# ayankele/dune-transformercvn

Hardware: AMD Instinct MI355X
Metric: events/sec (fwd+bwd) at batch=32, 8 prongs/event; fraction of MFMA roofline (higher is better)
Workload: dtype bf16; 1 GPU; TransformerCVN DenseNet [3,6,12,6,3] g32, fwd+loss+bwd, batch 32/GPU, 8 prongs/event, 3x400x280 maps, 6-layer encoder, dropout 0.1; global_batch=32, parallelism=dp1, precision=bf16

## Files before the change

### dune-transformercvn_amd/csrc/bwd1x1_fused.hip

```cpp
#include "tcvn_ops.h"
#include "prof.h"

namespace tcvn {

namespace {

constexpr int ROWS = 64;
constexpr int TILE = ROWS * 256;
constexpr int CLD = 132;
constexpr int OFF_E = 0;
constexpr int OFF_X = TILE;
constexpr int OFF_Y = 2 * TILE;
constexpr int OFF_C = 2 * TILE;
constexpr int OFF_TAB = OFF_C + ROWS * CLD * 4;
constexpr int SMEM_BYTES = OFF_TAB + 5 * 128 * 4;

typedef __attribute__((ext_vector_type(4))) short s16x4;

__device__ __forceinline__ bf16x8_t tr_frag(const char* smem_base, int off_lo, int off_hi) {
    typedef __attribute__((address_space(3))) s16x4* lds_p;
    const s16x4 lo = __builtin_amdgcn_ds_read_tr16_b64_v4i16((lds_p)(smem_base + off_lo));
    const s16x4 hi = __builtin_amdgcn_ds_read_tr16_b64_v4i16((lds_p)(smem_base + off_hi));
    struct { s16x4 a, b; } pr = {lo, hi};
    return __builtin_bit_cast(bf16x8_t, pr);
}

__device__ __forceinline__ void dma64(char* smem_base, int buf_off, const bf16* __restrict__ A, long lda, int K, int k0, long m0, long M,
                                      const char* __restrict__ zeros, int wave, int lane) {
    const int rsub = lane >> 4, slot = lane & 15;
#pragma unroll
    for (int i = 0; i < ROWS / 16; ++i) {
        const int rg = wave + 4 * i;
        const int r = rg * 4 + rsub;
        const int col = k0 + ((slot ^ swz16(r)) << 3);
        const long m = m0 + r;
        const char* src = (m < M && col < K) ? reinterpret_cast<const char*>(A + m * lda + col) : zeros + (slot << 4);
        __builtin_amdgcn_global_load_lds((const __attribute__((address_space(1))) void*)src,
                                         (__attribute__((address_space(3))) void*)(smem_base + buf_off + rg * 1024), 16, 0, 0);
    }
}

__global__ __launch_bounds__(256, 2) void k_bwd1x1_fused_bf16(const Bwd1x1Args g) {
    extern __shared__ __attribute__((aligned(16))) char smem[];
    float* Cs = reinterpret_cast<float*>(smem + OFF_C);
    double* red = reinterpret_cast<double*>(smem + OFF_C);
    float* csum = reinterpret_cast<float*>(smem + OFF_C + 4 * 128 * 3 * 8);
    float* tab = reinterpret_cast<float*>(smem + OFF_TAB);

    const int tid = threadIdx.x;
    const int N = g.cin, n0 = blockIdx.y * 128;
    const bf16* __restrict__ DU = reinterpret_cast<const bf16*>(g.DU);
    const bf16* __restrict__ Yp = reinterpret_cast<const bf16*>(g.Y);
    const bf16* __restrict__ Xp = reinterpret_cast<const bf16*>(g.Xin);
    bf16* __restrict__ Gp = reinterpret_cast<bf16*>(g.Gout);
    const char* __restrict__ zeros = reinterpret_cast<const char*>(g.zeros);
    const long mtiles = (g.M + ROWS - 1) / ROWS;
    const u16x8 z8 = {0, 0, 0, 0, 0, 0, 0, 0};

    const bool wave_live = n0 + (tid >> 6) * 32 < N;
    bf16x8_t bw[8];
    {
        const bf16* __restrict__ Wf = reinterpret_cast<const bf16*>(g.Wfrag) + (((long)(blockIdx.y * 4 + (tid >> 6)) * 8) * 64 + (tid & 63)) * 8;
#pragma unroll
        for (int i = 0; i < 8; ++i) {
            if (wave_live) bw[i] = *reinterpret_cast<const bf16x8_t*>(Wf + (long)i * 512);
            else
#pragma unroll
                for (int j = 0; j < 8; ++j) bw[i][j] = (__bf16)0.f;
        }
    }
    if (tid < 128) {
        const bool ok = n0 + tid < N;
        tab[tid] = g.PY[tid]; tab[128 + tid] = g.QY[tid];
        tab[256 + tid] = ok ? g.sc[n0 + tid] : 0.f; tab[384 + tid] = ok ? g.sh[n0 + tid] : 0.f; tab[512 + tid] = ok ? g.sl[n0 + tid] : 0.f;
    }
    float st1[8], st2[8], st3[8], cs[8];
#pragma unroll
    for (int j = 0; j < 8; ++j) { st1[j] = 0.f; st2[j] = 0.f; st3[j] = 0.f; cs[j] = 0.f; }
    const bool wj_live = n0 + ((tid >> 6) & 1) * 64 < N;
    f32x16 accW[2][2];
#pragma unroll
    for (int a = 0; a < 2; ++a)
#pragma unroll
        for (int b = 0; b < 2; ++b)
#pragma unroll
            for (int e = 0; e < 16; ++e) accW[a][b][e] = 0.f;

    const int col_chunk = tid & 15;
    const bool col_ok = n0 + col_chunk * 8 < N;
    const int col_rem = N - (n0 + col_chunk * 8);
    const int d_r0 = (tid >> 6) * 4 + ((tid & 63) >> 4);
    const int d_chunk = (tid & 15) ^ swz16(d_r0);
    const bool xchunk_ok = n0 + (d_chunk << 3) < N;
    const unsigned voffA = (unsigned)(d_r0 * 256 + (d_chunk << 4));
    const unsigned voffX = (unsigned)(d_r0 * (int)g.ldx * 2 + (d_chunk << 4));
    const unsigned voffG = (unsigned)(((tid >> 4) * (int)g.ldg + n0 + col_chunk * 8) * 2);
    if (!xchunk_ok) {
#pragma unroll
        for (int i = 0; i < ROWS / 16; ++i) *reinterpret_cast<u16x8*>(smem + OFF_X + ((tid >> 6) + 4 * i) * 1024 + (tid & 63) * 16) = z8;
    }
    u16x8 pgv[ROWS / 16];
#pragma unroll
    for (int i = 0; i < ROWS / 16; ++i) pgv[i] = z8;
    auto request = [&](long t) {
        const long m0 = t * ROWS;
        const int wave = tid >> 6, lane = tid & 63;
        if (m0 + ROWS <= g.M) {
            const char* bE = reinterpret_cast<const char*>(DU) + m0 * 256;
            const char* bY = reinterpret_cast<const char*>(Yp) + m0 * 256;
            const char* bX = reinterpret_cast<const char*>(Xp) + (m0 * g.ldx + n0) * 2;
            const char* bG = reinterpret_cast<const char*>(Gp) + m0 * g.ldg * 2;
#pragma unroll
            for (int i = 0; i < ROWS / 16; ++i)
                __builtin_amdgcn_global_load_lds((const __attribute__((address_space(1))) void*)(bE + i * 4096 + voffA),
                                                 (__attribute__((address_space(3))) void*)(smem + OFF_E + (wave + 4 * i) * 1024), 16, 0, 0);
#pragma unroll
            for (int i = 0; i < ROWS / 16; ++i)
                __builtin_amdgcn_global_load_lds((const __attribute__((address_space(1))) void*)(bY + i * 4096 + voffA),
                                                 (__attribute__((address_space(3))) void*)(smem + OFF_Y + (wave + 4 * i) * 1024), 16, 0, 0);
            if (xchunk_ok) {
#pragma unroll
                for (int i = 0; i < ROWS / 16; ++i)
                    __builtin_amdgcn_global_load_lds((const __attribute__((address_space(1))) void*)(bX + (long)i * 32 * g.ldx + voffX),
                                                     (__attribute__((address_space(3))) void*)(smem + OFF_X + (wave + 4 * i) * 1024), 16, 0, 0);
            }
            if (col_ok) {
#pragma unroll
                for (int i = 0; i < ROWS / 16; ++i) pgv[i] = *reinterpret_cast<const u16x8*>(bG + (long)i * 32 * g.ldg + voffG);
            }
        } else {
            dma64(smem, OFF_E, DU, 128, 128, 0, m0, g.M, zeros, wave, lane);
            dma64(smem, OFF_Y, Yp, 128, 128, 0, m0, g.M, zeros, wave, lane);
            if (xchunk_ok) dma64(smem, OFF_X, Xp, g.ldx, N, n0, m0, g.M, zeros, wave, lane);
            if (col_ok) {
#pragma unroll
                for (int i = 0; i < ROWS / 16; ++i) {
                    const long m = m0 + (tid >> 4) + 16 * i;
                    if (m < g.M) pgv[i] = *reinterpret_cast<const u16x8*>(Gp + m * g.ldg + n0 + col_chunk * 8);
                }
            }
        }
    };

    long mt = blockIdx.x;
    if (mt < mtiles) request(mt);
    for (; mt < mtiles; mt += gridDim.x) {
        const long m0 = mt * ROWS;
        asm volatile("s_waitcnt vmcnt(0)" ::: "memory");
        __syncthreads();
        int t_o = tid;
        asm volatile("" : "+v"(t_o));
        const int c8 = t_o & 15, c_r0 = t_o >> 4;
        const int e_off = c_r0 * 256 + ((c8 ^ swz16(c_r0)) << 4);
        auto tab8 = [&](int which, float (&v)[8]) {
            const float4 a = *reinterpret_cast<const float4*>(tab + which * 128 + c8 * 8), b = *reinterpret_cast<const float4*>(tab + which * 128 + c8 * 8 + 4);
            v[0] = a.x; v[1] = a.y; v[2] = a.z; v[3] = a.w; v[4] = b.x; v[5] = b.y; v[6] = b.z; v[7] = b.w;
        };
        {
            float pP[8], pQ[8];
            tab8(0, pP); tab8(1, pQ);
#pragma unroll
            for (int i = 0; i < ROWS / 16; ++i) {
                const int off = e_off + i * 4096;
                const u16x8 dv = *reinterpret_cast<const u16x8*>(smem + OFF_E + off);
                const u16x8 yv = *reinterpret_cast<const u16x8*>(smem + OFF_Y + off);
                const bool live = m0 + c_r0 + 16 * i < g.M;
                u16x8 o;
#pragma unroll
                for (int j = 0; j < 8; ++j) {
                    const float t = eff3(bf2f(dv[j]), pP[j], bf2f(yv[j]), pQ[j]);
                    o[j] = live ? f2bf(t) : (bf16)0;
                    cs[j] += bf2f(o[j]);
                }
                *reinterpret_cast<u16x8*>(smem + OFF_E + off) = o;
            }
        }
        __syncthreads();
        {
            const int lane = t_o & 63, wave = t_o >> 6;
            const int r = lane & 31, h = lane >> 5;
            f32x16 acc[2];
#pragma unroll
            for (int i = 0; i < 2; ++i)
#pragma unroll
                for (int e = 0; e < 16; ++e) acc[i][e] = 0.f;
            if (wave_live) {
                const int a_base = OFF_E + r * 256, w4 = (h ^ swz16(r)) << 4;
                auto afrag = [&](int ks, int i) {
                    return *reinterpret_cast<const bf16x8_t*>(smem + a_base + i * 8192 + (w4 ^ (ks << 5)));
                };
                bf16x8_t a0 = afrag(0, 0), a1 = afrag(0, 1);
#pragma unroll
                for (int ks = 0; ks < 8; ++ks) {
                    bf16x8_t b0 = a0, b1 = a1;
                    if (ks + 1 < 8) { b0 = afrag(ks + 1, 0); b1 = afrag(ks + 1, 1); }
                    acc[0] = __builtin_amdgcn_mfma_f32_32x32x16_bf16(a0, bw[ks], acc[0], 0, 0, 0);
                    acc[1] = __builtin_amdgcn_mfma_f32_32x32x16_bf16(a1, bw[ks], acc[1], 0, 0, 0);
                    a0 = b0; a1 = b1;
                    __builtin_amdgcn_sched_barrier(0);
                }
            }
            float* cw = Cs + 4 * h * CLD + wave * 32 + r;
#pragma unroll
            for (int i = 0; i < 2; ++i)
#pragma unroll
                for (int e = 0; e < 16; ++e) cw[(i * 32 + (e & 3) + 8 * (e >> 2)) * CLD] = acc[i][e];
        }
        __syncthreads();
        if (col_ok) {
            float csc[8], csh[8], csl[8];
            tab8(2, csc); tab8(3, csh); tab8(4, csl);
            const float* crow = Cs + c_r0 * CLD + c8 * 8;
            char* gbase = reinterpret_cast<char*>(Gp) + m0 * g.ldg * 2;
#pragma unroll
            for (int i = 0; i < ROWS / 16; ++i) {
                if (m0 + c_r0 + 16 * i < g.M) {
                    const int xoff = OFF_X + e_off + i * 4096;
                    u16x8 xv = *reinterpret_cast<const u16x8*>(smem + xoff);
                    if (col_rem < 8) {
#pragma unroll
                        for (int j = 0; j < 8; ++j) xv[j] = j < col_rem ? xv[j] : (bf16)0;
                    }
                    const float4 ca = *reinterpret_cast<const float4*>(crow + i * 16 * CLD);
                    const float4 cc = *reinterpret_cast<const float4*>(crow + i * 16 * CLD + 4);
                    const float cv[8] = {ca.x, ca.y, ca.z, ca.w, cc.x, cc.y, cc.z, cc.w};
                    const u16x8 gv = pgv[i];
                    u16x8 o, xa;
#pragma unroll
                    for (int j = 0; j < 8; ++j) {
                        const float x = bf2f(xv[j]);
                        const float u = fmaf(x, csc[j], csh[j]);
                        const float dA = cv[j];
                        const float du = u > 0.f ? dA : csl[j] * dA;
                        st1[j] += du; st2[j] = fmaf(du, x, st2[j]); st3[j] = fmaf(u > 0.f ? 0.f : dA, u, st3[j]);
                        o[j] = f2bf(fmaf(csc[j], du, bf2f(gv[j])));
                        xa[j] = f2bf(prelu(u, csl[j]));
                    }
                    if (col_rem >= 8) *reinterpret_cast<u16x8*>(gbase + (long)i * 32 * g.ldg + voffG) = o;
                    else {
                        bf16* gp = reinterpret_cast<bf16*>(gbase + (long)i * 32 * g.ldg + voffG);
#pragma unroll
                        for (int j = 0; j < 8; ++j)
                            if (j < col_rem) gp[j] = o[j];
                    }
                    *reinterpret_cast<u16x8*>(smem + xoff) = xa;
                }
            }
        }
        __syncthreads();
        if (wj_live) {
            const int lane = t_o & 63, wave = t_o >> 6;
            const int wi = wave >> 1, wj = wave & 1;
            const int gq = lane >> 4, tq = (lane >> 2) & 3, tp = lane & 3;
            const int khalf = gq >> 1, chalf = gq & 1;
            const int sub = (tp & 1) * 8;
            const int rl = 8 * khalf + tq;
            int a_lo[2], a_hi[2], b_lo[2], b_hi[2];
#pragma unroll
            for (int t = 0; t < 2; ++t) {
                const int ac = wi * 8 + t * 4 + 2 * chalf + (tp >> 1), bc = wj * 8 + t * 4 + 2 * chalf + (tp >> 1);
                a_lo[t] = OFF_E + rl * 256 + ((ac ^ swz16(rl)) << 4) + sub; a_hi[t] = OFF_E + (rl + 4) * 256 + ((ac ^ swz16(rl + 4)) << 4) + sub;
                b_lo[t] = OFF_X + rl * 256 + ((bc ^ swz16(rl)) << 4) + sub; b_hi[t] = OFF_X + (rl + 4) * 256 + ((bc ^ swz16(rl + 4)) << 4) + sub;
            }
#pragma unroll
            for (int ks = 0; ks < ROWS / 16; ++ks) {
                bf16x8_t a[2], b[2];
#pragma unroll
                for (int t = 0; t < 2; ++t) {
                    a[t] = tr_frag(smem, a_lo[t] + ks * 4096, a_hi[t] + ks * 4096);
                    b[t] = tr_frag(smem, b_lo[t] + ks * 4096, b_hi[t] + ks * 4096);
                }
#pragma unroll
                for (int ta = 0; ta < 2; ++ta)
#pragma unroll
                    for (int tb = 0; tb < 2; ++tb) accW[ta][tb] = __builtin_amdgcn_mfma_f32_32x32x16_bf16(a[ta], b[tb], accW[ta][tb], 0, 0, 0);
                __builtin_amdgcn_sched_barrier(0);
            }
        }
        __syncthreads();
        if (mt + gridDim.x < mtiles) request(mt + gridDim.x);
    }
    asm volatile("s_waitcnt vmcnt(0)" ::: "memory");

    const int lane = tid & 63, wave = tid >> 6, c8 = tid & 15;
#pragma unroll
    for (int j = 0; j < 8; ++j) {
        double d1 = (double)st1[j], d2 = (double)st2[j], d3 = (double)st3[j];
        float c1 = cs[j];
        d1 += __shfl_xor(d1, 16); d1 += __shfl_xor(d1, 32);
        d2 += __shfl_xor(d2, 16); d2 += __shfl_xor(d2, 32);
        d3 += __shfl_xor(d3, 16); d3 += __shfl_xor(d3, 32);
        c1 += __shfl_xor(c1, 16); c1 += __shfl_xor(c1, 32);
        if (lane < 16) {
            double* p = red + ((wave * 128) + c8 * 8 + j) * 3;
            p[0] = d1; p[1] = d2; p[2] = d3;
            csum[wave * 128 + c8 * 8 + j] = c1;
        }
    }
    __syncthreads();
    if (tid < 128) {
        if (n0 + tid < N) {
            double a = 0, b = 0, c = 0;
#pragma unroll
            for (int w = 0; w < 4; ++w) { a += red[(w * 128 + tid) * 3]; b += red[(w * 128 + tid) * 3 + 1]; c += red[(w * 128 + tid) * 3 + 2]; }
            double* p = g.part + ((long)blockIdx.x * N + n0 + tid) * 3;
            p[0] = a; p[1] = b; p[2] = c;
        }
        if (blockIdx.y == 0) g.tail[(long)blockIdx.x * 128 + tid] = (csum[tid] + csum[128 + tid]) + (csum[256 + tid] + csum[384 + tid]);
    }
    const int wi = wave >> 1, wj = wave & 1;
    const int cj = lane & 31, hh = lane >> 5;
#pragma unroll
    for (int ta = 0; ta < 2; ++ta)
#pragma unroll
        for (int tb = 0; tb < 2; ++tb) {
            const int j = n0 + wj * 64 + tb * 32 + cj;
            if (j >= g.ldc) continue;
#pragma unroll
            for (int e = 0; e < 16; ++e) {
                const int i = wi * 64 + ta * 32 + (e & 3) + 8 * (e >> 2) + 4 * hh;
                g.slab[((long)blockIdx.x * 128 + i) * g.ldc + j] = accW[ta][tb][e];
            }
        }
}

}

bool bwd1x1_fused_ok(const Bwd1x1Args& a) {
    if (!a.DU || !a.Y || !a.Xin || !a.Gout || !a.Wfrag || !a.zeros || !a.part || !a.slab || !a.tail) return false;
    if (a.cin <= 0 || a.Kp != 128 || (a.ldx & 7) || (a.ldg & 7) || a.ldc < a.cin || a.ldc > cdiv(a.cin, 128) * 128) return false;
    const uintptr_t al = reinterpret_cast<uintptr_t>(a.DU) | reinterpret_cast<uintptr_t>(a.Y) | reinterpret_cast<uintptr_t>(a.Xin) |
                         reinterpret_cast<uintptr_t>(a.Gout) | reinterpret_cast<uintptr_t>(a.Wfrag) | reinterpret_cast<uintptr_t>(a.slab);
    if (al & 15) return false;
    return (long)bwd1x1_fused_nblk(a) * 128 * a.ldc * 4 <= a.slab_bytes;
}

int bwd1x1_fused_nblk(const Bwd1x1Args& a) {
    const int nn = cdiv(a.cin, 128);
    int cap = 512 / nn;
    if (cap < 64) cap = 64;
    const long mt = (a.M + ROWS - 1) / ROWS;
    return (int)(mt < cap ? mt : cap);
}

int bwd1x1_fused_launch(const Bwd1x1Args& a, hipStream_t st) {
    if (a.M <= 0) return 0;
    if (!bwd1x1_fused_ok(a)) return -2;
    if (a.nblk != bwd1x1_fused_nblk(a)) { fprintf(stderr, "tcvn: bwd1x1_fused nblk mismatch\n"); return -3; }
    static bool attr = false;
    if (!attr) {
        TCVN_CHECK(hipFuncSetAttribute(reinterpret_cast<const void*>(k_bwd1x1_fused_bf16), hipFuncAttributeMaxDynamicSharedMemorySize, 160 * 1024));
        attr = true;
    }
    ProfScope ps("k_bwd1x1_fused_bf16", 4.0 * a.M * 128.0 * a.cin, (double)a.M * (512.0 + 4.0 * a.cin), st);
    hipLaunchKernelGGL(k_bwd1x1_fused_bf16, dim3(a.nblk, cdiv(a.cin, 128)), dim3(256), SMEM_BYTES, st, a);
    TCVN_LAUNCH_CHECK();
    return 0;
}

int bwd1x1_fused_reduce(const Bwd1x1Args& a, float* dWk, float* dbias, const SlabJob* extra, hipStream_t st, const BnBwdLinkArgs* link) {
    SlabJob jobs[4] = {};
    if (a.M > 0) { jobs[0] = slab_job(a.slab, a.nblk, 128L * a.ldc, dWk, 0); jobs[1] = slab_job(a.tail, a.nblk, 128, dbias, 0); }
    if (extra != nullptr) { jobs[2] = extra[0]; jobs[3] = extra[1]; }
    if (link != nullptr) return slab_reduce4_link(jobs, 4, *link, st);
    return slab_reduce4(jobs, 4, st);
}

}
```

### dune-transformercvn_amd/csrc/fwd1x1_fused.hip

```cpp
#include "tcvn_ops.h"
#include "prof.h"

namespace tcvn {

namespace {

constexpr int ROWS = 64;
constexpr int TILE = ROWS * 256;
constexpr int CLD = 136;

template <int NKC> struct FwdCfg {
    static constexpr int OFF_C = NKC * TILE;
    static constexpr int OFF_TAB = OFF_C + ROWS * CLD * 2;
    static constexpr int SMEM = OFF_TAB + 3 * NKC * 128 * 4;
};

template <int NKC, bool OACT>
__global__ __launch_bounds__(256, 3) void k_fwd1x1_fused_bf16(const Fwd1x1Args g) {
    extern __shared__ __attribute__((aligned(16))) char smem[];
    typedef FwdCfg<NKC> C;
    constexpr int KS = NKC * 8;
    bf16* Cs = reinterpret_cast<bf16*>(smem + C::OFF_C);
    double* red = reinterpret_cast<double*>(smem);
    float* tab = reinterpret_cast<float*>(smem + C::OFF_TAB);

    const int tid = threadIdx.x;
    const int K = g.cin;
    const bf16* __restrict__ Xp = reinterpret_cast<const bf16*>(g.Xin);
    const char* __restrict__ zeros = reinterpret_cast<const char*>(g.zeros);
    const long mtiles = (g.M + ROWS - 1) / ROWS;
    const int ksteps = g.Kp >> 4;
    const u16x8 z8 = {0, 0, 0, 0, 0, 0, 0, 0};

    bf16x8_t bw[KS];
    {
        const bf16* __restrict__ Wf = reinterpret_cast<const bf16*>(g.Wfrag) + (((long)(tid >> 6) * ksteps) * 64 + (tid & 63)) * 8;
#pragma unroll
        for (int i = 0; i < KS; ++i) {
            if (i < ksteps) bw[i] = *reinterpret_cast<const bf16x8_t*>(Wf + (long)i * 512);
            else
#pragma unroll
                for (int j = 0; j < 8; ++j) bw[i][j] = (__bf16)0.f;
        }
    }
    for (int i = tid; i < NKC * 128; i += 256) {
        const bool ok = i < K;
        float tsc = 0.f, tsh = 0.f;
        if (ok) {
            if (g.lf.isum != nullptr) lf_table(g.lf, i, blockIdx.x == 0, tsc, tsh);
            else { tsc = g.sc[i]; tsh = g.sh[i]; }
        }
        tab[i] = tsc; tab[NKC * 128 + i] = tsh; tab[2 * NKC * 128 + i] = ok ? g.sl[i] : 0.f;
    }
    const int ocol = (tid >> 6) * 32 + (tid & 31);
    const float cbias = g.bias[ocol];
    const float o_sc = OACT ? g.osc[ocol] : 1.f, o_sh = OACT ? g.osh[ocol] : 0.f, o_sl = OACT ? g.osl[ocol] : 1.f;
    float st1[8], st2[8];
#pragma unroll
    for (int j = 0; j < 8; ++j) { st1[j] = 0.f; st2[j] = 0.f; }

    const int d_r0 = (tid >> 6) * 4 + ((tid & 63) >> 4);
    const int d_chunk = (tid & 15) ^ (d_r0 & 15);
    const unsigned voffX = (unsigned)(d_r0 * (int)g.ldx * 2 + (d_chunk << 4));
#pragma unroll
    for (int kc = 0; kc < NKC; ++kc)
        if (kc * 128 + (d_chunk << 3) >= K) {
#pragma unroll
            for (int i = 0; i < ROWS / 16; ++i) *reinterpret_cast<u16x8*>(smem + kc * TILE + ((tid >> 6) + 4 * i) * 1024 + (tid & 63) * 16) = z8;
        }
    auto request = [&](long t) {
        const long m0 = t * ROWS;
        const int wave = tid >> 6, lane = tid & 63;
        if (m0 + ROWS <= g.M) {
            const char* bX = reinterpret_cast<const char*>(Xp) + m0 * g.ldx * 2;
#pragma unroll
            for (int kc = 0; kc < NKC; ++kc)
                if (kc * 128 + (d_chunk << 3) < K) {
#pragma unroll
                    for (int i = 0; i < ROWS / 16; ++i)
                        __builtin_amdgcn_global_load_lds((const __attribute__((address_space(1))) void*)(bX + kc * 256 + (long)i * 32 * g.ldx + voffX),
                                                         (__attribute__((address_space(3))) void*)(smem + kc * TILE + (wave + 4 * i) * 1024), 16, 0, 0);
                }
        } else {
            const int rsub = lane >> 4, slot = lane & 15;
#pragma unroll
            for (int kc = 0; kc < NKC; ++kc)
                if (kc * 128 + (d_chunk << 3) < K) {
#pragma unroll
                    for (int i = 0; i < ROWS / 16; ++i) {
                        const int rg = wave + 4 * i;
                        const long m = m0 + rg * 4 + rsub;
                        const char* src = m < g.M ? reinterpret_cast<const char*>(Xp + m * g.ldx + kc * 128 + (d_chunk << 3)) : zeros + (slot << 4);
                        __builtin_amdgcn_global_load_lds((const __attribute__((address_space(1))) void*)src,
                                                         (__attribute__((address_space(3))) void*)(smem + kc * TILE + rg * 1024), 16, 0, 0);
                    }
                }
        }
    };

    long mt = blockIdx.x;
    if (mt < mtiles) request(mt);
    for (; mt < mtiles; mt += gridDim.x) {
        const long m0 = mt * ROWS;
        asm volatile("s_waitcnt vmcnt(0)" ::: "memory");
        __syncthreads();
        int t_o = tid;
        asm volatile("" : "+v"(t_o));
        const int c8 = t_o & 15, c_r0 = t_o >> 4;
        const int e_off = c_r0 * 256 + ((c8 ^ (c_r0 & 15)) << 4);
#pragma unroll
        for (int kc = 0; kc < NKC; ++kc) {
            const int col = kc * 128 + c8 * 8;
            if (col < K) {
                const float* tp = tab + col;
                const float4 s0 = *reinterpret_cast<const float4*>(tp), s1 = *reinterpret_cast<const float4*>(tp + 4);
                const float4 h0 = *reinterpret_cast<const float4*>(tp + NKC * 128), h1 = *reinterpret_cast<const float4*>(tp + NKC * 128 + 4);
                const float4 l0 = *reinterpret_cast<const float4*>(tp + 2 * NKC * 128), l1 = *reinterpret_cast<const float4*>(tp + 2 * NKC * 128 + 4);
                const float sc[8] = {s0.x, s0.y, s0.z, s0.w, s1.x, s1.y, s1.z, s1.w};
                const float sh[8] = {h0.x, h0.y, h0.z, h0.w, h1.x, h1.y, h1.z, h1.w};
                const float sl[8] = {l0.x, l0.y, l0.z, l0.w, l1.x, l1.y, l1.z, l1.w};
                const int nrem = K - col;
#pragma unroll
                for (int i = 0; i < ROWS / 16; ++i) {
                    u16x8* p = reinterpret_cast<u16x8*>(smem + kc * TILE + e_off + i * 4096);
                    const u16x8 v = *p;
                    u16x8 o;
#pragma unroll
                    for (int j = 0; j < 8; ++j) o[j] = j < nrem ? f2bf(prelu(fmaf(bf2f(v[j]), sc[j], sh[j]), sl[j])) : (bf16)0;
                    *p = o;
                }
            }
        }
        __syncthreads();
        const int lane = t_o & 63, wave = t_o >> 6;
        const int r = lane & 31, h = lane >> 5;
        f32x16 acc[2];
#pragma unroll
        for (int i = 0; i < 2; ++i)
#pragma unroll
            for (int e = 0; e < 16; ++e) acc[i][e] = 0.f;
        {
            const int a_base = r * 256, w4 = (h ^ (r & 15)) << 4;
            auto afrag = [&](int s, int i) {
                return *reinterpret_cast<const bf16x8_t*>(smem + (s >> 3) * TILE + a_base + i * 8192 + (w4 ^ ((s & 7) << 5)));
            };
            bf16x8_t a0 = afrag(0, 0), a1 = afrag(0, 1);
#pragma unroll
            for (int s = 0; s < KS; ++s) {
                if (s < ksteps) {
                    bf16x8_t b0 = a0, b1 = a1;
                    if (s + 1 < KS && s + 1 < ksteps) { b0 = afrag(s + 1, 0); b1 = afrag(s + 1, 1); }
                    acc[0] = __builtin_amdgcn_mfma_f32_32x32x16_bf16(a0, bw[s], acc[0], 0, 0, 0);
                    acc[1] = __builtin_amdgcn_mfma_f32_32x32x16_bf16(a1, bw[s], acc[1], 0, 0, 0);
                    a0 = b0; a1 = b1;
                }
                __builtin_amdgcn_sched_barrier(0);
            }
        }
        __syncthreads();
        if (mt + gridDim.x < mtiles) request(mt + gridDim.x);
        {
            bf16* cw = Cs + 4 * h * CLD + wave * 32 + r;
#pragma unroll
            for (int i = 0; i < 2; ++i)
#pragma unroll
                for (int e = 0; e < 16; ++e) {
                    float v = acc[i][e] + cbias;
                    if (OACT) v = prelu(fmaf(v, o_sc, o_sh), o_sl);
                    cw[(i * 32 + (e & 3) + 8 * (e >> 2)) * CLD] = f2bf(v);
                }
        }
        __syncthreads();
        {
            const bf16* crow = Cs + c_r0 * CLD + c8 * 8;
            bf16* yb = reinterpret_cast<bf16*>(g.Out) + (m0 + c_r0) * 128 + c8 * 8;
#pragma unroll
            for (int i = 0; i < ROWS / 16; ++i) {
                if (m0 + c_r0 + 16 * i < g.M) {
                    const u16x8 o = *reinterpret_cast<const u16x8*>(crow + i * 16 * CLD);
#pragma unroll
                    for (int j = 0; j < 8; ++j) {
                        const float x = bf2f(o[j]);
                        st1[j] += x; st2[j] += x * x;
                    }
                    *reinterpret_cast<u16x8*>(yb + (long)i * 16 * 128) = o;
                }
            }
        }
    }
    asm volatile("s_waitcnt vmcnt(0)" ::: "memory");
    if (g.part == nullptr && g.isum_out == nullptr) return;
    __syncthreads();
    const int lane = tid & 63, wave = tid >> 6, c8 = tid & 15;
#pragma unroll
    for (int j = 0; j < 8; ++j) {
        double d1 = (double)st1[j], d2 = (double)st2[j];
        d1 += __shfl_xor(d1, 16); d1 += __shfl_xor(d1, 32);
        d2 += __shfl_xor(d2, 16); d2 += __shfl_xor(d2, 32);
        if (lane < 16) {
            double* p = red + ((wave * 128) + c8 * 8 + j) * 2;
            p[0] = d1; p[1] = d2;
        }
    }
    __syncthreads();
    if (tid < 128) {
        double a = 0, b = 0;
#pragma unroll
        for (int w = 0; w < 4; ++w) { a += red[(w * 128 + tid) * 2]; b += red[(w * 128 + tid) * 2 + 1]; }
        if (g.isum_out != nullptr) lf_add(g.isum_out, g.isum_stride, tid, a, b);
        else { double* p = g.part + ((long)blockIdx.x * 128 + tid) * 2; p[0] = a; p[1] = b; }
    }
}

struct WideCfg {
    static constexpr int NSLOT = 3;
    static constexpr int OFF_C = NSLOT * TILE;
    static constexpr int OFF_TAB = OFF_C + ROWS * CLD * 2;
    static constexpr int SMEM = OFF_TAB + 3 * 512 * 4;
};

template <bool OACT>
__global__ __launch_bounds__(256, 2) void k_fwd1x1_wide_bf16(const Fwd1x1Args g) {
    extern __shared__ __attribute__((aligned(16))) char smem[];
    constexpr int KS = 32;
    bf16* Cs = reinterpret_cast<bf16*>(smem + WideCfg::OFF_C);
    double* red = reinterpret_cast<double*>(smem);
    float* tab = reinterpret_cast<float*>(smem + WideCfg::OFF_TAB);

    const int tid = threadIdx.x;
    const int K = g.cin, nkc = (K + 127) >> 7;
    const bf16* __restrict__ Xp = reinterpret_cast<const bf16*>(g.Xin);
    const char* __restrict__ zeros = reinterpret_cast<const char*>(g.zeros);
    const long mtiles = (g.M + ROWS - 1) / ROWS;
    const int ksteps = g.Kp >> 4;

    for (int i = tid; i < 512; i += 256) {
        const bool ok = i < K;
        float tsc = 0.f, tsh = 0.f;
        if (ok) {
            if (g.lf.isum != nullptr) lf_table(g.lf, i, blockIdx.x == 0, tsc, tsh);
            else { tsc = g.sc[i]; tsh = g.sh[i]; }
        }
        tab[i] = tsc; tab[512 + i] = tsh; tab[1024 + i] = ok ? g.sl[i] : 0.f;
    }
    __syncthreads();
    bf16x8_t bw[KS];
    {
        const bf16* __restrict__ Wf = reinterpret_cast<const bf16*>(g.Wfrag) + (((long)(tid >> 6) * ksteps) * 64 + (tid & 63)) * 8;
#pragma unroll
        for (int i = 0; i < KS; ++i) {
            if (i < ksteps) bw[i] = *reinterpret_cast<const bf16x8_t*>(Wf + (long)i * 512);
            else
#pragma unroll
                for (int j = 0; j < 8; ++j) bw[i][j] = (__bf16)0.f;
        }
    }
    const int ocol = (tid >> 6) * 32 + (tid & 31);
    const float cbias = g.bias[ocol];
    const float o_sc = OACT ? g.osc[ocol] : 1.f, o_sh = OACT ? g.osh[ocol] : 0.f, o_sl = OACT ? g.osl[ocol] : 1.f;
    float st1[8], st2[8];
#pragma unroll
    for (int j = 0; j < 8; ++j) { st1[j] = 0.f; st2[j] = 0.f; }

    const int d_r0 = (tid >> 6) * 4 + ((tid & 63) >> 4);
    const int d_chunk = (tid & 15) ^ (d_r0 & 15);
    const unsigned voffX = (unsigned)(d_r0 * (int)g.ldx * 2 + (d_chunk << 4));
    auto request = [&](long t, int kc, int slot) {
        const long m0 = t * ROWS;
        const int wave = tid >> 6;
        const char* bX = reinterpret_cast<const char*>(Xp) + m0 * g.ldx * 2 + kc * 256;
        const bool colok = kc * 128 + (d_chunk << 3) < K;
#pragma unroll
        for (int i = 0; i < ROWS / 16; ++i) {
            const bool ok = colok && m0 + d_r0 + 16 * i < g.M;
            const char* src = ok ? bX + (long)i * 32 * g.ldx + voffX : zeros + ((tid & 15) << 4);
            __builtin_amdgcn_global_load_lds((const __attribute__((address_space(1))) void*)src,
                                             (__attribute__((address_space(3))) void*)(smem + slot * TILE + (wave + 4 * i) * 1024), 16, 0, 0);
        }
    };

    long r_mt = blockIdx.x;
    int r_kc = 0, r_slot = 0, inflight = 0;
    auto request_next = [&]() {
        if (r_mt >= mtiles) return;
        request(r_mt, r_kc, r_slot);
        ++inflight;
        if (++r_kc == nkc) { r_kc = 0; r_mt += gridDim.x; }
        r_slot = r_slot == WideCfg::NSLOT - 1 ? 0 : r_slot + 1;
    };
    __builtin_amdgcn_s_waitcnt(0x0F70);
    request_next();
    request_next();
    int slot = 0;
    for (long mt = blockIdx.x; mt < mtiles; mt += gridDim.x) {
        const long m0 = mt * ROWS;
        const bool first = mt == (long)blockIdx.x;
        int t_o = tid;
        asm volatile("" : "+v"(t_o));
        const int c8 = t_o & 15, c_r0 = t_o >> 4;
        const int e_off = c_r0 * 256 + ((c8 ^ (c_r0 & 15)) << 4);
        const int lane = t_o & 63, wave = t_o >> 6;
        const int r = lane & 31, h = lane >> 5;
        const int a_base = r * 256, w4 = (h ^ (r & 15)) << 4;
        f32x16 acc[2];
#pragma unroll
        for (int i = 0; i < 2; ++i)
#pragma unroll
            for (int e = 0; e < 16; ++e) acc[i][e] = 0.f;
#pragma unroll
        for (int kc = 0; kc < 4; ++kc) {
            if (kc < nkc) {
                if (inflight < 2) asm volatile("s_waitcnt vmcnt(0)" ::: "memory");
                else if (kc == 0 && !first) asm volatile("s_waitcnt vmcnt(8)" ::: "memory");
                else asm volatile("s_waitcnt vmcnt(4)" ::: "memory");
                asm volatile("s_barrier" ::: "memory");
                --inflight;
                request_next();
                const int col = kc * 128 + c8 * 8;
                if (col < K) {
                    const float* tp = tab + col;
                    const f32x4 s0 = *reinterpret_cast<const f32x4*>(tp), s1 = *reinterpret_cast<const f32x4*>(tp + 4);
                    const f32x4 h0 = *reinterpret_cast<const f32x4*>(tp + 512), h1 = *reinterpret_cast<const f32x4*>(tp + 516);
                    const f32x4 l0 = *reinterpret_cast<const f32x4*>(tp + 1024), l1 = *reinterpret_cast<const f32x4*>(tp + 1028);
                    const float sc[8] = {s0.x, s0.y, s0.z, s0.w, s1.x, s1.y, s1.z, s1.w};
                    const float sh[8] = {h0.x, h0.y, h0.z, h0.w, h1.x, h1.y, h1.z, h1.w};
                    const float sl[8] = {l0.x, l0.y, l0.z, l0.w, l1.x, l1.y, l1.z, l1.w};
                    const int nrem = K - col;
                    if (nrem >= 8) {
#pragma unroll
                        for (int i = 0; i < ROWS / 16; ++i) {
                            u16x8* p = reinterpret_cast<u16x8*>(smem + slot * TILE + e_off + i * 4096);
                            const u16x8 v = *p;
                            u16x8 o;
#pragma unroll
                            for (int j = 0; j < 8; ++j) o[j] = f2bf(prelu(fmaf(bf2f(v[j]), sc[j], sh[j]), sl[j]));
                            *p = o;
                        }
                    } else {
#pragma unroll
                        for (int i = 0; i < ROWS / 16; ++i) {
                            u16x8* p = reinterpret_cast<u16x8*>(smem + slot * TILE + e_off + i * 4096);
                            const u16x8 v = *p;
                            u16x8 o;
#pragma unroll
                            for (int j = 0; j < 8; ++j) o[j] = j < nrem ? f2bf(prelu(fmaf(bf2f(v[j]), sc[j], sh[j]), sl[j])) : (bf16)0;
                            *p = o;
                        }
                    }
                }
                asm volatile("s_waitcnt lgkmcnt(0)\n\ts_barrier" ::: "memory");
                auto afrag = [&](int ks, int i) {
                    return *reinterpret_cast<const bf16x8_t*>(smem + slot * TILE + a_base + i * 8192 + (w4 ^ (ks << 5)));
                };
                bf16x8_t a0 = afrag(0, 0), a1 = afrag(0, 1);
#pragma unroll
                for (int ks = 0; ks < 8; ++ks) {
                    bf16x8_t b0 = a0, b1 = a1;
                    if (ks + 1 < 8) { b0 = afrag(ks + 1, 0); b1 = afrag(ks + 1, 1); }
                    acc[0] = __builtin_amdgcn_mfma_f32_32x32x16_bf16(a0, bw[kc * 8 + ks], acc[0], 0, 0, 0);
                    acc[1] = __builtin_amdgcn_mfma_f32_32x32x16_bf16(a1, bw[kc * 8 + ks], acc[1], 0, 0, 0);
                    a0 = b0; a1 = b1;
                    __builtin_amdgcn_sched_barrier(0);
                }
                slot = slot == WideCfg::NSLOT - 1 ? 0 : slot + 1;
            }
        }
        {
            bf16* cw = Cs + 4 * h * CLD + wave * 32 + r;
#pragma unroll
            for (int i = 0; i < 2; ++i)
#pragma unroll
                for (int e = 0; e < 16; ++e) {
                    float v = acc[i][e] + cbias;
                    if (OACT) v = prelu(fmaf(v, o_sc, o_sh), o_sl);
                    cw[(i * 32 + (e & 3) + 8 * (e >> 2)) * CLD] = f2bf(v);
                }
        }
        asm volatile("s_waitcnt lgkmcnt(0)\n\ts_barrier" ::: "memory");
        {
            const bf16* crow = Cs + c_r0 * CLD + c8 * 8;
            bf16* yb = reinterpret_cast<bf16*>(g.Out) + (m0 + c_r0) * 128 + c8 * 8;
            auto row = [&](int i) {
                const u16x8 o = *reinterpret_cast<const u16x8*>(crow + i * 16 * CLD);
#pragma unroll
                for (int j = 0; j < 8; ++j) {
                    const float x = bf2f(o[j]);
                    st1[j] += x; st2[j] += x * x;
                }
                *reinterpret_cast<u16x8*>(yb + (long)i * 16 * 128) = o;
            };
            if (m0 + ROWS <= g.M) {
#pragma unroll
                for (int i = 0; i < ROWS / 16; ++i) row(i);
            } else {
#pragma unroll
                for (int i = 0; i < ROWS / 16; ++i)
                    if (m0 + c_r0 + 16 * i < g.M) row(i);
            }
        }
    }
    asm volatile("s_waitcnt vmcnt(0)" ::: "memory");
    if (g.part == nullptr && g.isum_out == nullptr) return;
    __syncthreads();
    const int lane = tid & 63, wave = tid >> 6, c8 = tid & 15;
#pragma unroll
    for (int j = 0; j < 8; ++j) {
        double d1 = (double)st1[j], d2 = (double)st2[j];
        d1 += __shfl_xor(d1, 16); d1 += __shfl_xor(d1, 32);
        d2 += __shfl_xor(d2, 16); d2 += __shfl_xor(d2, 32);
        if (lane < 16) {
            double* p = red + ((wave * 128) + c8 * 8 + j) * 2;
            p[0] = d1; p[1] = d2;
        }
    }
    __syncthreads();
    if (tid < 128) {
        double a = 0, b = 0;
#pragma unroll
        for (int w = 0; w < 4; ++w) { a += red[(w * 128 + tid) * 2]; b += red[(w * 128 + tid) * 2 + 1]; }
        if (g.isum_out != nullptr) lf_add(g.isum_out, g.isum_stride, tid, a, b);
        else { double* p = g.part + ((long)blockIdx.x * 128 + tid) * 2; p[0] = a; p[1] = b; }
    }
}

}

bool fwd1x1_fused_ok(const Fwd1x1Args& a) {
    if (!a.Xin || !a.Out || !a.Wfrag || !a.zeros || !a.bias || !a.sl) return false;
    if (a.lf.isum == nullptr && (!a.sc || !a.sh)) return false;
    if (a.lf.isum != nullptr && (!a.lf.bstat || !a.lf.gamma || !a.lf.beta || !a.lf.sc_out || !a.lf.sh_out || a.lf.count <= 0)) return false;
    if (a.isum_out != nullptr && a.osc != nullptr) return false;
    if (a.osc != nullptr && (a.part != nullptr || !a.osh || !a.osl)) return false;
    if (a.cin <= 0 || a.cin > 512 || a.Kp < a.cin || a.Kp > 512 || (a.Kp & 15) || (a.ldx & 7) || a.ldx < a.cin) return false;
    const uintptr_t al = reinterpret_cast<uintptr_t>(a.Xin) | reinterpret_cast<uintptr_t>(a.Out) | reinterpret_cast<uintptr_t>(a.Wfrag);
    return (al & 15) == 0;
}

int fwd1x1_fused_nblk(const Fwd1x1Args& a) {
    constexpr int CAP = 768, CAP_WIDE = 512;
    static_assert(CAP <= LF_MAX_ADDERS && CAP_WIDE <= LF_MAX_ADDERS, "bn_lf.h: more workgroups would add to one channel than its range guard allows for");
    const int cap = a.Kp <= 256 ? CAP : CAP_WIDE;
    const long mt = (a.M + ROWS - 1) / ROWS;
    return (int)(mt < cap ? mt : cap);
}

int fwd1x1_fused(const Fwd1x1Args& a, hipStream_t st) {
    if (a.M <= 0) return 0;
    if (!fwd1x1_fused_ok(a)) return -2;
    if (a.part != nullptr && a.isum_out == nullptr && a.nblk != fwd1x1_fused_nblk(a)) { fprintf(stderr, "tcvn: fwd1x1_fused nblk mismatch\n"); return -3; }
    static bool attr = false;
    if (!attr) {
        const void* fns[4] = {reinterpret_cast<const void*>(k_fwd1x1_fused_bf16<1, false>), reinterpret_cast<const void*>(k_fwd1x1_fused_bf16<2, false>),
                              reinterpret_cast<const void*>(k_fwd1x1_fused_bf16<1, true>), reinterpret_cast<const void*>(k_fwd1x1_fused_bf16<2, true>)};
        for (const void* f : fns) TCVN_CHECK(hipFuncSetAttribute(f, hipFuncAttributeMaxDynamicSharedMemorySize, 160 * 1024));
        TCVN_CHECK(hipFuncSetAttribute(reinterpret_cast<const void*>(k_fwd1x1_wide_bf16<false>), hipFuncAttributeMaxDynamicSharedMemorySize, 160 * 1024));
        TCVN_CHECK(hipFuncSetAttribute(reinterpret_cast<const void*>(k_fwd1x1_wide_bf16<true>), hipFuncAttributeMaxDynamicSharedMemorySize, 160 * 1024));
        attr = true;
    }
    ProfScope ps("k_fwd1x1_fused_bf16", 2.0 * a.M * 128.0 * a.cin, (double)a.M * 2.0 * (a.cin + 128.0), st);
    const int nblk = fwd1x1_fused_nblk(a);
    const bool oact = a.osc != nullptr;
    if (a.Kp > 256 && oact) hipLaunchKernelGGL(k_fwd1x1_wide_bf16<true>, dim3(nblk), dim3(256), WideCfg::SMEM, st, a);
    else if (a.Kp > 256) hipLaunchKernelGGL(k_fwd1x1_wide_bf16<false>, dim3(nblk), dim3(256), WideCfg::SMEM, st, a);
    else if (a.Kp <= 128 && oact) hipLaunchKernelGGL((k_fwd1x1_fused_bf16<1, true>), dim3(nblk), dim3(256), FwdCfg<1>::SMEM, st, a);
    else if (a.Kp <= 128) hipLaunchKernelGGL((k_fwd1x1_fused_bf16<1, false>), dim3(nblk), dim3(256), FwdCfg<1>::SMEM, st, a);
    else if (oact) hipLaunchKernelGGL((k_fwd1x1_fused_bf16<2, true>), dim3(nblk), dim3(256), FwdCfg<2>::SMEM, st, a);
    else hipLaunchKernelGGL((k_fwd1x1_fused_bf16<2, false>), dim3(nblk), dim3(256), FwdCfg<2>::SMEM, st, a);
    TCVN_LAUNCH_CHECK();
    return 0;
}

}
```

Baseline: 1807 events/s.

## Split bwd1x1 prefetch into two stages and replace syncthreads with targeted waits

Splits the per-tile prefetch in the fused backward 1x1 kernel into two groups. Y and G are now requested before the weight-gradient MFMA phase, and E and X after it, so loads overlap more compute. Full __syncthreads calls are replaced with explicit s_waitcnt/s_barrier sequences that wait only on the needed counters, and transpose LDS reads use inline asm with a single lgkmcnt wait. The kernel is also templated on whether cin is a multiple of 8 and whether a tile is full, which removes bounds masking on the common path. The hand-written waitcnt values (vmcnt(4)) are fragile and risk hazards if the load counts change.

```diff
diff --git a/dune-transformercvn_amd/csrc/bwd1x1_fused.hip b/dune-transformercvn_amd/csrc/bwd1x1_fused.hip
--- a/dune-transformercvn_amd/csrc/bwd1x1_fused.hip
+++ b/dune-transformercvn_amd/csrc/bwd1x1_fused.hip
@@ -1,5 +1,6 @@
 #include "tcvn_ops.h"
 #include "prof.h"
+#include <type_traits>
 
 namespace tcvn {
 
@@ -17,12 +18,15 @@
 
 typedef __attribute__((ext_vector_type(4))) short s16x4;
 
-__device__ __forceinline__ bf16x8_t tr_frag(const char* smem_base, int off_lo, int off_hi) {
-    typedef __attribute__((address_space(3))) s16x4* lds_p;
-    const s16x4 lo = __builtin_amdgcn_ds_read_tr16_b64_v4i16((lds_p)(smem_base + off_lo));
-    const s16x4 hi = __builtin_amdgcn_ds_read_tr16_b64_v4i16((lds_p)(smem_base + off_hi));
+__device__ __forceinline__ bf16x8_t tr_frag_asm(unsigned a_lo, unsigned a_hi, int off) {
+    s16x4 lo, hi;
+    asm volatile("ds_read_b64_tr_b16 %0, %1 offset:%2" : "=v"(lo) : "v"(a_lo), "i"(off) : "memory");
+    asm volatile("ds_read_b64_tr_b16 %0, %1 offset:%2" : "=v"(hi) : "v"(a_hi), "i"(off) : "memory");
     struct { s16x4 a, b; } pr = {lo, hi};
     return __builtin_bit_cast(bf16x8_t, pr);
+}
+__device__ __forceinline__ void tr_wait(bf16x8_t& a0, bf16x8_t& a1, bf16x8_t& b0, bf16x8_t& b1) {
+    asm volatile("s_waitcnt lgkmcnt(0)" : "+v"(a0), "+v"(a1), "+v"(b0), "+v"(b1) :: "memory");
 }
 
 __device__ __forceinline__ void dma64(char* smem_base, int buf_off, const bf16* __restrict__ A, long lda, int K, int k0, long m0, long M,
@@ -40,6 +44,7 @@
     }
 }
 
+template <bool FULLC>
 __global__ __launch_bounds__(256, 2) void k_bwd1x1_fused_bf16(const Bwd1x1Args g) {
     extern __shared__ __attribute__((aligned(16))) char smem[];
     float* Cs = reinterpret_cast<float*>(smem + OFF_C);
@@ -94,7 +99,7 @@
     const bool xchunk_ok = n0 + (d_chunk << 3) < N;
     const unsigned voffA = (unsigned)(d_r0 * 256 + (d_chunk << 4));
     const unsigned voffX = (unsigned)(d_r0 * (int)g.ldx * 2 + (d_chunk << 4));
-    const unsigned voffG = (unsigned)(((tid >> 4) * (int)g.ldg + n0 + col_chunk * 8) * 2);
+    const unsigned voffG = (unsigned)(((tid >> 4) * (int)g.ldg + n0 + (col_ok ? col_chunk : 0) * 8) * 2);
     if (!xchunk_ok) {
 #pragma unroll
         for (int i = 0; i < ROWS / 16; ++i) *reinterpret_cast<u16x8*>(smem + OFF_X + ((tid >> 6) + 4 * i) * 1024 + (tid & 63) * 16) = z8;
@@ -102,58 +107,66 @@
     u16x8 pgv[ROWS / 16];
 #pragma unroll
     for (int i = 0; i < ROWS / 16; ++i) pgv[i] = z8;
-    auto request = [&](long t) {
+    auto request_yg = [&](long t) {
         const long m0 = t * ROWS;
-        const int wave = tid >> 6, lane = tid & 63;
+        const int wave = tid >> 6;
+        if (m0 + ROWS <= g.M) {
+            const char* bY = reinterpret_cast<const char*>(Yp) + m0 * 256;
+            const char* bG = reinterpret_cast<const char*>(Gp) + m0 * g.ldg * 2;
+#pragma unroll
+            for (int i = 0; i < ROWS / 16; ++i)
+                __builtin_amdgcn_global_load_lds((const __attribute__((address_space(1))) void*)(bY + i * 4096 + voffA),
+                                                 (__attribute__((address_space(3))) void*)(smem + OFF_Y + (wave + 4 * i) * 1024), 16, 0, 0);
+#pragma unroll
+            for (int i = 0; i < ROWS / 16; ++i) pgv[i] = *reinterpret_cast<const u16x8*>(bG + (long)i * 32 * g.ldg + voffG);
+        } else {
+            int t_p = tid;
+            asm volatile("" : "+v"(t_p));
+            dma64(smem, OFF_Y, Yp, 128, 128, 0, m0, g.M, zeros, t_p >> 6, t_p & 63);
+#pragma unroll
+            for (int i = 0; i < ROWS / 16; ++i) {
+                const long m = m0 + (t_p >> 4) + 16 * i;
+                pgv[i] = *reinterpret_cast<const u16x8*>(Gp + (m < g.M ? m : g.M - 1) * g.ldg + n0 + (col_ok ? t_p & 15 : 0) * 8);
+            }
+        }
+    };
+    auto request_ex = [&](long t) {
+        const long m0 = t * ROWS;
+        const int wave = tid >> 6;
         if (m0 + ROWS <= g.M) {
             const char* bE = reinterpret_cast<const char*>(DU) + m0 * 256;
-            const char* bY = reinterpret_cast<const char*>(Yp) + m0 * 256;
             const char* bX = reinterpret_cast<const char*>(Xp) + (m0 * g.ldx + n0) * 2;
-            const char* bG = reinterpret_cast<const char*>(Gp) + m0 * g.ldg * 2;
 #pragma unroll
             for (int i = 0; i < ROWS / 16; ++i)
                 __builtin_amdgcn_global_load_lds((const __attribute__((address_space(1))) void*)(bE + i * 4096 + voffA),
                                                  (__attribute__((address_space(3))) void*)(smem + OFF_E + (wave + 4 * i) * 1024), 16, 0, 0);
-#pragma unroll
-            for (int i = 0; i < ROWS / 16; ++i)
-                __builtin_amdgcn_global_load_lds((const __attribute__((address_space(1))) void*)(bY + i * 4096 + voffA),
-                                                 (__attribute__((address_space(3))) void*)(smem + OFF_Y + (wave + 4 * i) * 1024), 16, 0, 0);
             if (xchunk_ok) {
 #pragma unroll
                 for (int i = 0; i < ROWS / 16; ++i)
                     __builtin_amdgcn_global_load_lds((const __attribute__((address_space(1))) void*)(bX + (long)i * 32 * g.ldx + voffX),
                                                      (__attribute__((address_space(3))) void*)(smem + OFF_X + (wave + 4 * i) * 1024), 16, 0, 0);
             }
-            if (col_ok) {
-#pragma unroll
-                for (int i = 0; i < ROWS / 16; ++i) pgv[i] = *reinterpret_cast<const u16x8*>(bG + (long)i * 32 * g.ldg + voffG);
-            }
         } else {
-            dma64(smem, OFF_E, DU, 128, 128, 0, m0, g.M, zeros, wave, lane);
-            dma64(smem, OFF_Y, Yp, 128, 128, 0, m0, g.M, zeros, wave, lane);
-            if (xchunk_ok) dma64(smem, OFF_X, Xp, g.ldx, N, n0, m0, g.M, zeros, wave, lane);
-            if (col_ok) {
-#pragma unroll
-                for (int i = 0; i < ROWS / 16; ++i) {
-                    const long m = m0 + (tid >> 4) + 16 * i;
-                    if (m < g.M) pgv[i] = *reinterpret_cast<const u16x8*>(Gp + m * g.ldg + n0 + col_chunk * 8);
-                }
-            }
+            int t_p = tid;
+            asm volatile("" : "+v"(t_p));
+            dma64(smem, OFF_E, DU, 128, 128, 0, m0, g.M, zeros, t_p >> 6, t_p & 63);
+            if (xchunk_ok) dma64(smem, OFF_X, Xp, g.ldx, N, n0, m0, g.M, zeros, t_p >> 6, t_p & 63);
         }
     };
 
-    long mt = blockIdx.x;
-    if (mt < mtiles) request(mt);
-    for (; mt < mtiles; mt += gridDim.x) {
+    __builtin_amdgcn_s_waitcnt(0x0F70);
+    if ((long)blockIdx.x < mtiles) { request_yg(blockIdx.x); request_ex(blockIdx.x); }
+    auto trip = [&](auto full_tile, long mt) {
+        constexpr bool FT = decltype(full_tile)::value;
         const long m0 = mt * ROWS;
-        asm volatile("s_waitcnt vmcnt(0)" ::: "memory");
-        __syncthreads();
+        const bool more = mt + gridDim.x < mtiles;
+        asm volatile("s_waitcnt vmcnt(4) lgkmcnt(0)\n\ts_barrier" ::: "memory");
         int t_o = tid;
         asm volatile("" : "+v"(t_o));
         const int c8 = t_o & 15, c_r0 = t_o >> 4;
         const int e_off = c_r0 * 256 + ((c8 ^ swz16(c_r0)) << 4);
         auto tab8 = [&](int which, float (&v)[8]) {
-            const float4 a = *reinterpret_cast<const float4*>(tab + which * 128 + c8 * 8), b = *reinterpret_cast<const float4*>(tab + which * 128 + c8 * 8 + 4);
+            const f32x4 a = *reinterpret_cast<const f32x4*>(tab + which * 128 + c8 * 8), b = *reinterpret_cast<const f32x4*>(tab + which * 128 + c8 * 8 + 4);
             v[0] = a.x; v[1] = a.y; v[2] = a.z; v[3] = a.w; v[4] = b.x; v[5] = b.y; v[6] = b.z; v[7] = b.w;
         };
         {
@@ -164,18 +177,24 @@
                 const int off = e_off + i * 4096;
                 const u16x8 dv = *reinterpret_cast<const u16x8*>(smem + OFF_E + off);
                 const u16x8 yv = *reinterpret_cast<const u16x8*>(smem + OFF_Y + off);
-                const bool live = m0 + c_r0 + 16 * i < g.M;
+                const bool live = FT || m0 + c_r0 + 16 * i < g.M;
                 u16x8 o;
 #pragma unroll
                 for (int j = 0; j < 8; ++j) {
                     const float t = eff3(bf2f(dv[j]), pP[j], bf2f(yv[j]), pQ[j]);
-                    o[j] = live ? f2bf(t) : (bf16)0;
+                    if constexpr (FT) o[j] = f2bf(t);
+                    else o[j] = live ? f2bf(t) : (bf16)0;
                     cs[j] += bf2f(o[j]);
                 }
                 *reinterpret_cast<u16x8*>(smem + OFF_E + off) = o;
-            }
-        }
-        __syncthreads();
+                if constexpr (FT) {
+#pragma unroll
+                    for (int j = 0; j < 8; ++j) asm volatile("" : "+v"(cs[j]));
+                    __builtin_amdgcn_sched_barrier(0);
+                }
+            }
+        }
+        asm volatile("s_waitcnt lgkmcnt(0)\n\ts_barrier" ::: "memory");
         {
             const int lane = t_o & 63, wave = t_o >> 6;
             const int r = lane & 31, h = lane >> 5;
@@ -206,7 +225,7 @@
 #pragma unroll
                 for (int e = 0; e < 16; ++e) cw[(i * 32 + (e & 3) + 8 * (e >> 2)) * CLD] = acc[i][e];
         }
-        __syncthreads();
+        asm volatile("s_waitcnt vmcnt(0) lgkmcnt(0)\n\ts_barrier" ::: "memory");
         if (col_ok) {
             float csc[8], csh[8], csl[8];
             tab8(2, csc); tab8(3, csh); tab8(4, csl);
@@ -214,15 +233,17 @@
             char* gbase = reinterpret_cast<char*>(Gp) + m0 * g.ldg * 2;
 #pragma unroll
             for (int i = 0; i < ROWS / 16; ++i) {
-                if (m0 + c_r0 + 16 * i < g.M) {
+                if (FT || m0 + c_r0 + 16 * i < g.M) {
                     const int xoff = OFF_X + e_off + i * 4096;
                     u16x8 xv = *reinterpret_cast<const u16x8*>(smem + xoff);
-                    if (col_rem < 8) {
-#pragma unroll
-                        for (int j = 0; j < 8; ++j) xv[j] = j < col_rem ? xv[j] : (bf16)0;
+                    if constexpr (!FULLC) {
+                        if (col_rem < 8) {
+#pragma unroll
+                            for (int j = 0; j < 8; ++j) xv[j] = j < col_rem ? xv[j] : (bf16)0;
+                        }
                     }
-                    const float4 ca = *reinterpret_cast<const float4*>(crow + i * 16 * CLD);
-                    const float4 cc = *reinterpret_cast<const float4*>(crow + i * 16 * CLD + 4);
+                    const f32x4 ca = *reinterpret_cast<const f32x4*>(crow + i * 16 * CLD);
+                    const f32x4 cc = *reinterpret_cast<const f32x4*>(crow + i * 16 * CLD + 4);
                     const float cv[8] = {ca.x, ca.y, ca.z, ca.w, cc.x, cc.y, cc.z, cc.w};
                     const u16x8 gv = pgv[i];
                     u16x8 o, xa;
@@ -236,7 +257,7 @@
                         o[j] = f2bf(fmaf(csc[j], du, bf2f(gv[j])));
                         xa[j] = f2bf(prelu(u, csl[j]));
                     }
-                    if (col_rem >= 8) *reinterpret_cast<u16x8*>(gbase + (long)i * 32 * g.ldg + voffG) = o;
+                    if (FULLC || col_rem >= 8) *reinterpret_cast<u16x8*>(gbase + (long)i * 32 * g.ldg + voffG) = o;
                     else {
                         bf16* gp = reinterpret_cast<bf16*>(gbase + (long)i * 32 * g.ldg + voffG);
 #pragma unroll
@@ -245,9 +266,15 @@
                     }
                     *reinterpret_cast<u16x8*>(smem + xoff) = xa;
                 }
-            }
-        }
-        __syncthreads();
+                if constexpr (FT) {
+#pragma unroll
+                    for (int j = 0; j < 8; ++j) asm volatile("" : "+v"(st1[j]), "+v"(st2[j]), "+v"(st3[j]));
+                    __builtin_amdgcn_sched_barrier(0);
+                }
+            }
+        }
+        asm volatile("s_waitcnt lgkmcnt(0)\n\ts_barrier" ::: "memory");
+        if (more) request_yg(mt + gridDim.x);
         if (wj_live) {
             const int lane = t_o & 63, wave = t_o >> 6;
             const int wi = wave >> 1, wj = wave & 1;
@@ -255,7 +282,8 @@
             const int khalf = gq >> 1, chalf = gq & 1;
             const int sub = (tp & 1) * 8;
             const int rl = 8 * khalf + tq;
-            int a_lo[2], a_hi[2], b_lo[2], b_hi[2];
+            const unsigned lds0 = (unsigned)reinterpret_cast<size_t>((__attribute__((address_space(3))) char*)smem);
+            unsigned a_lo[2], a_hi[2], b_lo[2], b_hi[2];
 #pragma unroll
             for (int t = 0; t < 2; ++t) {
                 const int ac = wi * 8 + t * 4 + 2 * chalf + (tp >> 1), bc = wj * 8 + t * 4 + 2 * chalf + (tp >> 1);
@@ -267,9 +295,10 @@
                 bf16x8_t a[2], b[2];
 #pragma unroll
                 for (int t = 0; t < 2; ++t) {
-                    a[t] = tr_frag(smem, a_lo[t] + ks * 4096, a_hi[t] + ks * 4096);
-                    b[t] = tr_frag(smem, b_lo[t] + ks * 4096, b_hi[t] + ks * 4096);
-                }
+                    a[t] = tr_frag_asm(lds0 + a_lo[t], lds0 + a_hi[t], ks * 4096);
+                    b[t] = tr_frag_asm(lds0 + b_lo[t], lds0 + b_hi[t], ks * 4096);
+                }
+                tr_wait(a[0], a[1], b[0], b[1]);
 #pragma unroll
                 for (int ta = 0; ta < 2; ++ta)
 #pragma unroll
@@ -277,8 +306,15 @@
                 __builtin_amdgcn_sched_barrier(0);
             }
         }
-        __syncthreads();
-        if (mt + gridDim.x < mtiles) request(mt + gridDim.x);
+        asm volatile("s_waitcnt lgkmcnt(0)\n\ts_barrier" ::: "memory");
+        if (more) request_ex(mt + gridDim.x);
+    };
+    long mt = blockIdx.x;
+    if constexpr (FULLC) {
+        for (; mt * ROWS + ROWS <= g.M; mt += gridDim.x) trip(std::true_type{}, mt);
+        if (mt < mtiles) trip(std::false_type{}, mt);
+    } else {
+        for (; mt < mtiles; mt += gridDim.x) trip(std::false_type{}, mt);
     }
     asm volatile("s_waitcnt vmcnt(0)" ::: "memory");
 
@@ -349,11 +385,13 @@
     if (a.nblk != bwd1x1_fused_nblk(a)) { fprintf(stderr, "tcvn: bwd1x1_fused nblk mismatch\n"); return -3; }
     static bool attr = false;
     if (!attr) {
-        TCVN_CHECK(hipFuncSetAttribute(reinterpret_cast<const void*>(k_bwd1x1_fused_bf16), hipFuncAttributeMaxDynamicSharedMemorySize, 160 * 1024));
+        TCVN_CHECK(hipFuncSetAttribute(reinterpret_cast<const void*>(k_bwd1x1_fused_bf16<true>), hipFuncAttributeMaxDynamicSharedMemorySize, 160 * 1024));
+        TCVN_CHECK(hipFuncSetAttribute(reinterpret_cast<const void*>(k_bwd1x1_fused_bf16<false>), hipFuncAttributeMaxDynamicSharedMemorySize, 160 * 1024));
         attr = true;
     }
     ProfScope ps("k_bwd1x1_fused_bf16", 4.0 * a.M * 128.0 * a.cin, (double)a.M * (512.0 + 4.0 * a.cin), st);
-    hipLaunchKernelGGL(k_bwd1x1_fused_bf16, dim3(a.nblk, cdiv(a.cin, 128)), dim3(256), SMEM_BYTES, st, a);
+    if (a.cin % 8 == 0) hipLaunchKernelGGL(k_bwd1x1_fused_bf16<true>, dim3(a.nblk, cdiv(a.cin, 128)), dim3(256), SMEM_BYTES, st, a);
+    else hipLaunchKernelGGL(k_bwd1x1_fused_bf16<false>, dim3(a.nblk, cdiv(a.cin, 128)), dim3(256), SMEM_BYTES, st, a);
     TCVN_LAUNCH_CHECK();
     return 0;
 }
diff --git a/dune-transformercvn_amd/csrc/fwd1x1_fused.hip b/dune-transformercvn_amd/csrc/fwd1x1_fused.hip
--- a/dune-transformercvn_amd/csrc/fwd1x1_fused.hip
+++ b/dune-transformercvn_amd/csrc/fwd1x1_fused.hip
@@ -170,7 +170,7 @@
                     cw[(i * 32 + (e & 3) + 8 * (e >> 2)) * CLD] = f2bf(v);
                 }
         }
-        __syncthreads();
+        asm volatile("s_waitcnt lgkmcnt(0)\n\ts_barrier" ::: "memory");
         {
             const bf16* crow = Cs + c_r0 * CLD + c8 * 8;
             bf16* yb = reinterpret_cast<bf16*>(g.Out) + (m0 + c_r0) * 128 + c8 * 8;
```

Measured after the change: 1840 events/s, median of 6. +1.8%, better.
